# killerwhile/kafka-assignment-optimizer

Hardware: AMD Instinct MI355X
Metric: candidate assignments/sec (+ time_to_optimal_s), 10k-partition reassign (higher is better)
Workload: dtype int32

## Files before the change

kafka_assignment_optimizer_amd/csrc/kao_search.hip:

```cpp
#include "kao_search_dev.h"

namespace kao {

template <bool kGlobalA, bool kPriced, int NW, bool kWide, bool kTeam, bool kCurG = false, int RFT = 0, bool kSmall = false>
__device__ __forceinline__ void search_body(unsigned char *smem, const SearchPools &pl, const SearchParams &prm) {
    static_assert(!kTeam || kGlobalA, "teams run topics that live in global memory");
    static_assert(!kCurG || !kGlobalA, "kCurG: the working assignment is in LDS");
    static_assert(RFT == 0 || (RFT == 3 && NW == 4 && !kGlobalA && !kTeam), "RFT = 3: LDS-resident topics of four words per partition");
    static_assert(!kSmall || (RFT == 3 && !kPriced && !kCurG), "kSmall: the unpriced RF-3 instantiation");
    constexpr int NS = RFT ? RFT : NW;
    const int lane = threadIdx.x & 63;
    const int wave = __builtin_amdgcn_readfirstlane(threadIdx.x >> 6);
    const int n_waves = kTeam ? __builtin_amdgcn_readfirstlane((int)(blockDim.x >> 6)) : 1;
    const int tid = kTeam ? (int)threadIdx.x : lane, nthr = kTeam ? (int)blockDim.x : 64;
    const int2 bm = pl.block_map[blockIdx.x];
    const TopicDev *TD = pl.topics + bm.x;

    TopicRegs T = topic_regs<RFT>(TD);
    constexpr bool kBandTabs = kSmall;
    int bq_r0 = kBandTabs ? band_tab_bias(T.rep_lo) : T.rep_lo, bq_r1 = kBandTabs ? (int)band_tab(T.rep_lo, T.rep_hi) : T.rep_hi;
    int bq_l0 = kBandTabs ? band_tab_bias(T.lead_lo) : T.lead_lo, bq_l1 = kBandTabs ? (int)band_tab(T.lead_lo, T.lead_hi) : T.lead_hi;
    asm volatile("" : "+v"(bq_r0), "+v"(bq_r1), "+v"(bq_l0), "+v"(bq_l1));

    const int a_bytes = kGlobalA ? 0 : prm.maxP * NW * 4;
    const int cur_bytes = (kGlobalA || kCurG) ? 0 : prm.maxP * NW * 4;
    const int bx64 = (prm.maxBx + 63) & ~63;
    const int c_bytes = bx64 * 4;
    const int krt = search_rack_tab(prm.maxR);
    int *RSZ = reinterpret_cast<int *>(smem + cur_bytes);
    uint8_t *XR = smem + cur_bytes + krt * 4;
    const uint32_t inv = (uint32_t)krt - 1u;
    uint32_t *PR = reinterpret_cast<uint32_t *>(smem + cur_bytes + krt * 4 + bx64);
    const bool hbw = kPriced && prm.bw != 0;
    const int pr_bytes = kPriced ? (hbw ? 2 : 1) * c_bytes + krt * 4 : 0;
    int *PG = reinterpret_cast<int *>(smem + cur_bytes + krt * 4 + bx64 + c_bytes);
    uint32_t *BW = reinterpret_cast<uint32_t *>(smem + cur_bytes + krt * 4 + bx64 + c_bytes + krt * 4);
    unsigned char *wb = smem + cur_bytes + krt * 4 + bx64 + pr_bytes + (kTeam ? 0 : wave * (a_bytes + c_bytes + c_bytes / 2 + krt * 8));
    const Part<NW> *cur_words = reinterpret_cast<const Part<NW> *>(pl.cur_pool + TD->cur_off);
    const Part<NW> *CUR;
    if (kGlobalA || kCurG) CUR = cur_words; else CUR = reinterpret_cast<const Part<NW> *>(smem);
    WaveLds<NW> L;
    L.C = reinterpret_cast<uint32_t *>(wb + a_bytes);
    L.W = reinterpret_cast<uint16_t *>(wb + a_bytes + c_bytes);
    L.K = reinterpret_cast<int *>(wb + a_bytes + c_bytes + c_bytes / 2);
    L.RT = L.K + krt + (kTeam ? wave * krt : 0);
    int *TR = L.K + krt + n_waves * krt;
    int *TS = TR + 2 * 16 * kTeamRec;

    if (!kGlobalA && !kCurG) {
        Part<NW> *cur_lds = reinterpret_cast<Part<NW> *>(smem);
        for (int p = threadIdx.x; p < T.P; p += blockDim.x) cur_lds[p] = cur_words[p];
    }
    for (int r = threadIdx.x; r < krt; r += blockDim.x) {
        RSZ[r] = r < T.R ? pl.rsz_pool[TD->rsz_off + r] : 0;
        if (kPriced) PG[r] = r < T.R ? price_units(pl.price_pool[TD->price_off + 2 * TD->B + r], prm.obj_scale) : 0;
    }
    __syncthreads();
    for (int x = threadIdx.x; x < ((T.Bx + 63) & ~63); x += blockDim.x) {
        const uint32_t r = mulhi((uint32_t)x, T.magic);
        const bool valid = x < T.Bx && (int)((uint32_t)x - r * (uint32_t)T.m) < RSZ[r < (uint32_t)krt ? r : 0];
        XR[x] = valid ? (uint8_t)r : (uint8_t)inv;
        if (kPriced) {
            uint32_t pr = 0;
            if (valid) {
                const int32_t *pp = pl.price_pool + TD->price_off;
                const int b = pl.ext_pool[TD->ext_off + x];
                pr = ((uint32_t)price_units(pp[b], prm.obj_scale) & 0xFFFFu) | ((uint32_t)price_units(pp[TD->B + b], prm.obj_scale) << 16);
            }
            PR[x] = pr;
            if (hbw) BW[x] = (valid && TD->has_bw) ? pl.bw_pool[TD->bw_off + x] : 0u;
        }
    }
    __syncthreads();

    const int rho = bm.y + (kTeam ? 0 : wave);
    if (rho >= TD->n_restarts) return;
    const int g = TD->restart_base + rho;
    unsigned char *state_packed = pl.state_pool + TD->state_off + (uint64_t)rho * T.P * (NW * 2);
    if (kGlobalA) L.A = reinterpret_cast<Part<NW> *>(pl.state_pool + TD->state_off) + (uint64_t)rho * T.P;
    else L.A = reinterpret_cast<Part<NW> *>(wb);
    uint16_t *best = pl.best_pool + TD->best_off + (uint64_t)rho * T.P * T.RF;
    const uint16_t *ext = pl.ext_pool + TD->ext_off;
    const uint32_t slo = TD->seed_lo, shi = TD->seed_hi;
    const int S = prm.obj_scale;

    int best_obj, accepted;
    if (prm.init) {
        if (prm.init == 1)
        for (int p = tid; p < T.P; p += nthr) {
            Part<NW> c = CUR[p];
#pragma unroll
            for (int k = 1; k < NW; ++k)
                if (k >= T.RF) c.w[k] = kNoneW;
            L.A[p] = c;
        }
        best_obj = -1; accepted = 0;
    } else {
        best_obj = pl.restart_info[g * 4 + 0];
        accepted = pl.restart_info[g * 4 + 3];
        bool reseed = false;
        if (prm.elite) {
            const unsigned long long ek = pl.elite_key[bm.x];
            const int e_obj = (int)kObjCap - (int)((ek >> 20) & 0xFFFFFFull);
            reseed = ek != ~0ull && (ek >> 44) == 0 && (int)(ek & 0xFFFFFull) != rho && best_obj < e_obj &&
                     (fmix32(slo ^ ((uint32_t)rho * 0x9E3779B1u) ^ (prm.launch * 0x85EBCA77u) ^ 0xE117Eu) & 1u);
        }
        if (reseed) {
            const uint16_t *ea = pl.elite_assign + TD->win_off;
            const uint16_t *io = pl.int_pool + TD->int_off;
            for (int p = tid; p < T.P; p += nthr) {
                Part<NW> w;
#pragma unroll
                for (int k = 0; k < NW; ++k) w.w[k] = k < T.RF ? to_word(T, io[ea[p * T.RF + k]]) : kNoneW;
                L.A[p] = w;
            }
        } else if (!kGlobalA) {
            for (int p = lane; p < T.P; p += 64) L.A[p] = load_packed<NW>(T, state_packed, p);
        }
    }
    if (kGlobalA) __builtin_amdgcn_fence(__ATOMIC_SEQ_CST, "workgroup");
    if (kTeam) __syncthreads();
    recount(T, L, tid, nthr, krt);
    if (kTeam) __syncthreads();

    if (prm.init == 1) {
        const uint32_t *HL = pl.cur_pool + TD->hole_off;
        if (!kTeam || wave == 0)
        for (int pass = 0; pass < 2; ++pass) {
            const uint32_t n_holes = HL[pass], *hl = HL + 2 + (pass ? HL[0] : 0u);
            int p_n = n_holes ? (int)hl[0] : 0;
            Part<NW> a_n = L.A[p_n], c_n = CUR[p_n];
            for (uint32_t hi = 0; hi < n_holes; ++hi) {
                const int p = p_n;
                Part<NW> a = a_n;
                const Part<NW> c = c_n;
                if (hi + 1 < n_holes) { p_n = (int)hl[hi + 1]; a_n = L.A[p_n]; c_n = CUR[p_n]; }
#pragma unroll
                for (int k = 0; k < NW; ++k) {
                    if (k >= T.RF) break;
                    if ((k == 0) != (pass == 0)) continue;
                    if (a.w[k] != kNoneW) continue;
                    const uint32_t hmix = slo ^ fmix32(shi + (uint32_t)rho * 0x9E3779B1u + (uint32_t)(p * NW + k) * 0x27D4EB2Fu + 0x5BD1E995u + prm.gen * 0x632BE5ABu);
                    const int wl = k == 0 ? T.w00 : T.w01, wf = k == 0 ? T.w10 : T.w11;
                    uint32_t key = kKeyNull, xw_l = kNoneW;
#pragma unroll 2
                    for (int base = 0; base < T.Bx; base += 64) {
                        const uint32_t x = (uint32_t)(base + lane);
                        const uint32_t r = XR[x];
                        const uint32_t xw = x | (r << 16);
                        const bool okx = (r != inv) & !in4(a, xw);
                        const uint32_t cn = L.C[x];
                        const uint32_t rk = r;
                        int dV = dinc((int)(cn & 0xFFFFu), T.rep_lo, T.rep_hi) + dinc(L.K[rk], T.rack_lo, T.rack_hi) +
                                 dinc(cnt4(a, r), T.prack_lo, T.prack_hi);
                        if (k == 0) dV += dinc((int)(cn >> 16), T.lead_lo, T.lead_hi);
                        const uint32_t tie = fmix32(hmix + x * 0x165667B1u) >> 24;
                        uint32_t keyx;
                        if (kPriced) {
                            const uint32_t prx = PR[x];
                            int dP = p_in((int)(cn & 0xFFFFu), T.rep_lo, T.rep_hi, price_rep(prx)) + p_in(L.K[rk], T.rack_lo, T.rack_hi, PG[rk]);
                            if (k == 0) dP += p_in((int)(cn >> 16), T.lead_lo, T.lead_hi, price_lead(prx));
                            keyx = okx ? make_key_tie_p(prm.lam_max, S, dV, role_w2(c, xw, wl, wf) + (hbw ? bw_of(BW[x], k == 0) : 0), dP, tie) : kKeyNull;
                        }
                        else keyx = okx ? make_key_tie(prm.lam_max, S, dV, role_w2(c, xw, wl, wf), tie) : kKeyNull;
                        if (keyx < key) { key = keyx; xw_l = xw; }
                    }
                    const uint32_t kmin = wave_umin(key);
                    const unsigned long long bal = __ballot(key == kmin);
                    const uint32_t xw_win = (uint32_t)__builtin_amdgcn_readlane((int)xw_l, __ffsll((long long)bal) - 1);
                    a.w[k] = xw_win;
                    if (lane == 0) {
                        reinterpret_cast<uint32_t *>(&L.A[p])[k] = xw_win;
                        L.C[xw_win & 0xFFFFu] += (k == 0) ? 0x10001u : 1u;
                        L.K[xw_win >> 16] += 1;
                    }
                }
            }
        }
        if (kGlobalA) __builtin_amdgcn_fence(__ATOMIC_SEQ_CST, "workgroup");
        if (kTeam) __syncthreads();
    }

    int V, obj;
    full_cost<NW, kTeam>(T, L, CUR, RSZ, tid, nthr, V, obj, hbw ? BW : nullptr, TS, wave, n_waves);
    if (V == 0 && obj > best_obj) { best_obj = obj; snapshot(T, L, ext, best, tid, nthr); }
    rebuild_band_state(T, L, XR, inv, tid, nthr);
    if (lane == 0) L.RT[krt - 1] = 0;
    if (kTeam) __syncthreads();

    uint32_t rng = fmix32(slo ^ fmix32(shi + (uint32_t)rho * 0x9E3779B1u + prm.launch * 0x85EBCA77u + (uint32_t)tid * 0xC2B2AE3Du));

    const int plog = TD->period_log2 + (rho & 3);
    const uint32_t pmask = (1u << plog) - 1u;
    const uint32_t lrange = (uint32_t)(prm.lam_max - prm.lam_min + 1);
    const uint32_t RF8 = (uint32_t)T.RF << 8, R8 = (uint32_t)T.R << 8, m8 = (uint32_t)T.m << 8;

    const int T_tour = min(64, max(4, (T.P * T.RF) >> 2));
    uint32_t tour_off = lane < T_tour ? 0u : kKeyNull;
    asm volatile("" : "+v"(tour_off));
    const int GA = min(16, max(1, (T.P * T.RF) >> 8));
    const int x_rounds_full = (T.P + 63) >> 6;
    const bool x_windowed = x_rounds_full > 8;

    int lam_lo = prm.lam_min, lam_hi = prm.lam_max;
    uint32_t n_iters = prm.iters, it_base = prm.launch * prm.iters;
    constexpr uint32_t kLpScanTwo = 1u << 29;
    uint32_t loop_pack = TD->P * TD->RF <= prm.scan2_max ? kLpScanTwo : 0u;
    if (kSmall) loop_pack |= ((uint32_t)prm.lam_min & 0xFFFu) | (((uint32_t)prm.lam_max & 0xFFFu) << 12) | (((uint32_t)plog & 31u) << 24);
    {
        uint32_t v0 = (uint32_t)lam_lo, v1 = (uint32_t)lam_hi, v2 = n_iters, v3 = it_base, v4 = loop_pack;
        asm volatile("" : "+v"(v2), "+v"(v3), "+v"(v4));
        if constexpr (!kSmall) {
            asm volatile("" : "+v"(v0), "+v"(v1));
            lam_lo = (int)__builtin_amdgcn_readfirstlane(v0); lam_hi = (int)__builtin_amdgcn_readfirstlane(v1);
        }
        n_iters = __builtin_amdgcn_readfirstlane(v2); it_base = __builtin_amdgcn_readfirstlane(v3);
        loop_pack = __builtin_amdgcn_readfirstlane(v4);
    }
    auto loop_flag = [&](uint32_t bit) { uint32_t lp = loop_pack; asm volatile("" : "+s"(lp)); return (lp & bit) != 0u; };
    constexpr bool kFuse = !kGlobalA && !kTeam && !kPriced;
    const bool fuse_ok = kFuse && T.Bx <= 16384;
    uint32_t jmp_a = 1u, jmp_c = 0u;
    if (fuse_ok)
        for (int n = (T.Bx + 63) >> 6; n > 0; --n) { jmp_a = (jmp_a * 0x6D2B79u) & 0xFFFFFFu; jmp_c = (jmp_c * 0x6D2B79u + 0x3C6EF3u) & 0xFFFFFFu; }
    best_obj = __builtin_amdgcn_readfirstlane(best_obj);
    for (uint32_t i = 0; i < n_iters; ++i) {
        const uint32_t it = it_base + i;
        const int type = (int)((0x1210u >> ((it & 7u) * 2u)) & 3u);
        int lam;
        if constexpr (kSmall) {
            uint32_t lp = loop_pack;
            asm volatile("" : "+s"(lp));
            const uint32_t plg = (lp >> 24) & 31u;
            const int lo_ = (int)(lp & 0xFFFu), hi_ = (int)((lp >> 12) & 0xFFFu);
            const uint32_t ph = it & ((1u << plg) - 1u);
            lam = best_obj < 0 ? hi_ : min(hi_, lo_ + (int)((2u * ph * (uint32_t)(hi_ - lo_ + 1)) >> plg));
        } else {
            const uint32_t ph = it & pmask;
            lam = best_obj < 0 ? lam_hi : min(lam_hi, lam_lo + (int)((2u * ph * lrange) >> plog));
        }
        const bool sampled = (type == 2) || (type == 0 && ((it >> 3) & 1u));

        auto finish = [&](auto ty, auto uni, uint32_t kmin, int win, int p, int k, int q, int j, uint32_t uw, uint32_t vw, int dV, int dObj) {
            constexpr int TY = decltype(ty)::value;
            auto of_win = [&](int v) { return decltype(uni)::value ? v : __builtin_amdgcn_readlane(v, win); };
            if (!kTeam) {
                if (kmin == kKeyNull) return;
                if ((int)(kmin >> 8) - kDBias > 0) return;
            }
            bool mine = true;
            int *rec = TR + ((i & 1u) * 16 + (uint32_t)wave) * kTeamRec;
            if (kTeam) {
                const bool ok = kmin != kKeyNull && (int)(kmin >> 8) - kDBias <= 0;
                if (lane == win) {
                    const uint32_t ro_ = uw >> 16, rn_ = vw >> 16;
                    const bool racks = ok && TY == 0 && ro_ != rn_;
                    rec[0] = ok ? 1 : 0; rec[1] = p; rec[2] = TY == 1 ? q : p;
                    rec[3] = (int)(uw & 0xFFFFu); rec[4] = (int)(vw & 0xFFFFu);
                    rec[5] = racks ? (int)ro_ : 0xFFFF; rec[6] = racks ? (int)rn_ : 0xFFFF;
                    rec[7] = dV; rec[8] = dObj;
                }
                __syncthreads();
                bool clash = false;
                if (lane < wave) {
                    const int *o = TR + ((i & 1u) * 16 + (uint32_t)lane) * kTeamRec;
                    if (o[0]) {
                        const int mp = rec[1], mq = rec[2], mb0 = rec[3], mb1 = rec[4], mr0 = rec[5], mr1 = rec[6];
                        clash = (o[1] == mp) | (o[1] == mq) | (o[2] == mp) | (o[2] == mq) | (o[3] == mb0) | (o[3] == mb1) | (o[4] == mb0) | (o[4] == mb1);
                        if (o[5] != 0xFFFF && mr0 != 0xFFFF) clash |= (o[5] == mr0) | (o[5] == mr1) | (o[6] == mr0) | (o[6] == mr1);
                    }
                }
                mine = ok && __ballot(clash) == 0ull;
            }

            if (lane == win && mine) {
                uint32_t *ap = reinterpret_cast<uint32_t *>(&L.A[p]);
                if (TY == 0) {
                    const uint32_t d = (k == 0) ? 0x10001u : 1u;
                    L.C[uw & 0xFFFFu] -= d;
                    L.C[vw & 0xFFFFu] += d;
                    if (!kTeam || (uw >> 16) != (vw >> 16)) {
                        L.K[uw >> 16] -= 1;
                        L.K[vw >> 16] += 1;
                    }
                    ap[k] = vw;
                } else if (TY == 1) {
                    uint32_t *bp = reinterpret_cast<uint32_t *>(&L.A[q]);
                    if ((k == 0) != (j == 0)) {
                        const uint32_t lose = (k == 0) ? uw : vw, gain = (k == 0) ? vw : uw;
                        L.C[lose & 0xFFFFu] -= 0x10000u;
                        L.C[gain & 0xFFFFu] += 0x10000u;
                    }
                    ap[k] = vw;
                    bp[j] = uw;
                } else {
                    L.C[uw & 0xFFFFu] -= 0x10000u;
                    L.C[vw & 0xFFFFu] += 0x10000u;
                    ap[0] = vw;
                    ap[k] = uw;
                }
            }
            if (mine) {
                int rows;
                if (TY == 0) rows = 1 | (of_win(k) == 0 ? 2 : 0);
                else if (TY == 1) rows = (of_win(k) == 0 ? 2 : 0) ^ (of_win(j) == 0 ? 2 : 0);
                else rows = 2;
                if (rows != 0) {
                    const uint32_t xo = (uint32_t)of_win((int)uw) & 0xFFFFu, xn = decltype(uni)::value ? (uint32_t)__builtin_amdgcn_readfirstlane((int)(vw & 0xFFFFu)) : (uint32_t)of_win((int)vw) & 0xFFFFu;
                    uint32_t xx = xo;
                    asm("v_writelane_b32 %0, %1, 1" : "+v"(xx) : "s"(xn));
                    int lane_w = lane;
                    asm volatile("" : "+v"(lane_w));
                    if (lane_w < 2) {
                        const uint32_t cx = L.C[xx];
                        uint32_t wx;
                        if (rows == 3) wx = band_row<kBandTabs>((int)(cx & 0xFFFFu), bq_r0, bq_r1) | (band_row<kBandTabs>((int)(cx >> 16), bq_l0, bq_l1) << 6);
                        else if (rows == 1) wx = (L.W[xx] & ~kWRowR) | band_row<kBandTabs>((int)(cx & 0xFFFFu), bq_r0, bq_r1);
                        else wx = (L.W[xx] & ~kWRowL) | (band_row<kBandTabs>((int)(cx >> 16), bq_l0, bq_l1) << 6);
                        L.W[xx] = (uint16_t)wx;
                    }
                }
            }
            if (kGlobalA) __builtin_amdgcn_fence(__ATOMIC_SEQ_CST, "workgroup");
            if (kTeam) {
                if (lane == 0) rec[9] = mine ? 1 : 0;
                __syncthreads();
                int dVs = 0, dOs = 0, na = 0;
                if (lane < n_waves) {
                    const int *o = TR + ((i & 1u) * 16 + (uint32_t)lane) * kTeamRec;
                    if (o[9]) { dVs = o[7]; dOs = o[8]; na = 1; }
                }
                V += wave_sum(dVs);
                obj += wave_sum(dOs);
                accepted += wave_sum(na);
            } else {
                V += of_win(dV);
                obj += of_win(dObj);
                accepted++;
            }
        };
        constexpr std::integral_constant<int, 0> kReplace{};
        constexpr std::integral_constant<int, 1> kExchange{};
        constexpr std::integral_constant<int, 2> kLeaderSwap{};

        if (sampled) {
            const int p = (int)rnd24_wide(rng, (uint32_t)T.P);
            const Part<NW> a = L.A[p];
            const Part<NW> c = CUR[p];
            uint32_t key = kKeyNull, vw = 0;
            int dV = 0, dObj = 0;
            if (type == 0) {
                const int k = (int)rnd24(rng, RF8);
                const uint32_t uw = sel_slot<NS>(a, k);
                const uint32_t ro = uw >> 16;
                const bool lead = k == 0;
                const uint32_t lw = lead ? 2u : 0u;
                const int wl = lead ? T.w00 : T.w01, wf = lead ? T.w10 : T.w11;
                const int g_old = role_w2<NS>(c, uw, wl, wf) + (hbw ? bw_of(BW[uw & 0xFFFFu], lead) : 0);
                const uint32_t wo = L.W[uw & 0xFFFFu];
                const int dV_old = wfld(wo, kWDecR) + wfldw(wo, kWDecL, lw);
                const int dV_rack_old = ddec(L.K[ro], T.rack_lo, T.rack_hi) + c7_delta(T.c7_dec, cnt4x2<NS>(a, ro));
                const int rsz_ro = RSZ[ro];
                int dP_old = 0, dP_rack_old = 0;
                if (kPriced) {
                    const uint32_t pro = PR[uw & 0xFFFFu];
                    dP_old = -(wflag(wo, kWPoutR) & price_rep(pro));
                    if (lead) dP_old -= wflag(wo, kWPoutL) & price_lead(pro);
                    dP_rack_old = p_out(L.K[ro], T.rack_lo, T.rack_hi, PG[ro]);
                }
                const int base_s = kSmall ? mad24s(S, g_old, kDBias) : 0;
#pragma unroll
                for (int g = 0; g < 4; ++g) {
                    uint32_t r, jj;
                    bool okg;
                    if (g < 2) {
                        r = rnd24(rng, R8);
                        jj = rnd24(rng, m8);
                        okg = (int)jj < RSZ[r];
                    } else {
                        r = ro;
                        jj = rnd24(rng, (uint32_t)rsz_ro << 8);
                        okg = true;
                    }
                    const uint32_t x = __umul24(r, (uint32_t)T.m) + jj;
                    const uint32_t xw = x | (r << 16);
                    okg = okg && !in4<NS>(a, xw);
                    const uint32_t wn = L.W[x];
                    int dVg = dV_old + wfld(wn, kWIncR) + wfldw(wn, kWIncL, lw);
                    if (g < 2) {
                        if (r != ro)
                            dVg += dV_rack_old + dinc(L.K[r], T.rack_lo, T.rack_hi) + c7_delta(T.c7_inc, cnt4x2<NS>(a, r));
                    }
                    const int dObjg = role_w2<NS>(c, xw, wl, wf) + (hbw ? bw_of(BW[x], lead) : 0) - (kSmall ? 0 : g_old);
                    uint32_t keyg;
                    if constexpr (kSmall) keyg = okg ? key_small(mad24s(-S, dObjg, mad24s(lam, dVg, base_s)), (uint32_t)lane) : kKeyNull;
                    else if (kPriced) {
                        const uint32_t prx = PR[x];
                        int dPg = dP_old + (wflag(wn, kWPinR) & price_rep(prx));
                        if (lead) dPg += wflag(wn, kWPinL) & price_lead(prx);
                        if (g < 2 && r != ro) dPg += dP_rack_old + p_in(L.K[r], T.rack_lo, T.rack_hi, PG[r]);
                        keyg = okg ? make_key_p(lam, S, dVg, dObjg, dPg, lane) : kKeyNull;
                    }
                    else keyg = okg ? make_key(lam, S, dVg, dObjg, lane) : kKeyNull;
                    if (keyg < key) { key = keyg; vw = xw; dV = dVg; dObj = dObjg; }
                }
                if constexpr (kSmall) dObj -= g_old;
                const uint32_t kmin = wave_umin(key);
                finish(kReplace, std::false_type{}, kmin, (int)(kmin & 63u), p, k, 0, 0, uw, vw, dV, dObj);
            } else {
                const uint32_t uw = a.w[0];
                int k = 0;
                const int u_lead = role_w2<NS>(c, uw, T.w00, T.w10), u_fol = role_w2<NS>(c, uw, T.w01, T.w11);
                const uint32_t wu = L.W[uw & 0xFFFFu];
                const int dV_u = wfld(wu, kWDecL);
                const int dP_u = kPriced ? -(wflag(wu, kWPoutL) & price_lead(PR[uw & 0xFFFFu])) : 0;
#pragma unroll
                for (int kk = 1; kk < NS; ++kk) {
                    if (!RFT && kk >= T.RF) break;
                    const uint32_t xw = a.w[kk];
                    const int dObjg = role_w2<NS>(c, xw, T.w00, T.w10) + u_fol - u_lead - role_w2<NS>(c, xw, T.w01, T.w11) +
                                      (hbw ? (int)(BW[xw & 0xFFFFu] >> 16) - (int)(BW[uw & 0xFFFFu] >> 16) : 0);
                    const uint32_t wx = L.W[xw & 0xFFFFu];
                    const int dVg = dV_u + wfld(wx, kWIncL);
                    uint32_t keyg;
                    if constexpr (kSmall) keyg = key_small(mad24s(lam, dVg, mad24s(-S, dObjg, kDBias)), (uint32_t)lane);
                    else if (kPriced) keyg = make_key_p(lam, S, dVg, dObjg, dP_u + (wflag(wx, kWPinL) & price_lead(PR[xw & 0xFFFFu])), lane);
                    else keyg = make_key(lam, S, dVg, dObjg, lane);
                    if (keyg < key) { key = keyg; vw = xw; k = kk; dV = dVg; dObj = dObjg; }
                }
                const uint32_t kmin = wave_umin(key);
                finish(kLeaderSwap, std::false_type{}, kmin, (int)(kmin & 63u), p, k, 0, 0, uw, vw, dV, dObj);
            }
        } else {
            uint32_t keyA, oldw_l;
            int pl_, kl_, g_old_l, dvo_l = 0, dvr_l = 0;
            auto score_words = [&](auto ty, uint32_t &key_o, const Part<NW> &al, const Part<NW> &cl, int k_o, uint32_t &oldw_o, int &g_o, int &dvo_o, int &dvr_o) {
                constexpr int TY = decltype(ty)::value;
                oldw_o = sel_slot<NS>(al, k_o);
                const uint32_t rol = oldw_o >> 16;
                const bool leadl = k_o == 0;
                g_o = role_w2<NS>(cl, oldw_o, leadl ? T.w00 : T.w01, leadl ? T.w10 : T.w11);
                if (hbw && TY == 0) g_o += bw_of(BW[oldw_o & 0xFFFFu], leadl);
                const uint32_t wo = L.W[oldw_o & 0xFFFFu];
                const int dv7 = c7_delta(T.c7_dec, cnt4x2<NS>(al, rol));
                int sc;
                if (TY == 0) {
                    dvo_o = wfld(wo, kWDecR) + wfldw(wo, kWDecL, leadl ? 2u : 0u);
                    dvr_o = ddec(L.K[rol], T.rack_lo, T.rack_hi) + dv7;
                    sc = dvo_o + min(dvr_o, 0);
                } else {
                    const int dvl = wfld(wo, leadl ? kWDecL : kWIncL);
                    sc = min(dv7, 0) + min(dvl, 0);
                }
                if constexpr (kSmall) key_o = key_small(mad24s(lam, sc, mad24s(S, g_o, kDBias)), (uint32_t)lane) | tour_off;
                else if (kPriced) {
                    int dPs = 0;
                    if (TY == 0) {
                        const uint32_t pro = PR[oldw_o & 0xFFFFu];
                        dPs = -(wflag(wo, kWPoutR) & price_rep(pro));
                        dPs -= wflagw(wo, kWPoutL, leadl ? 1u : 0u) & price_lead(pro);
                    }
                    key_o = make_key_p(lam, S, sc, -g_o, dPs, lane) | tour_off;
                }
                else key_o = make_key(lam, S, sc, -g_o, lane) | tour_off;
            };
            auto score_slot = [&](auto ty, uint32_t &key_o, int p_o, int &k_o, uint32_t &oldw_o, int &g_o, int &dvo_o, int &dvr_o) {
                k_o = (int)rnd24(rng, RF8);
                const Part<NW> al = L.A[p_o];
                const Part<NW> cl = CUR[p_o];
                score_words(ty, key_o, al, cl, k_o, oldw_o, g_o, dvo_o, dvr_o);
            };
            auto tournament = [&](auto ty) {
                const int p0 = (int)rnd24_wide(rng, (uint32_t)T.P);
                auto part = [&](int ga) { const int q2 = p0 + ga; return q2 < T.P ? q2 : q2 - T.P; };
                pl_ = p0;
                score_slot(ty, keyA, p0, kl_, oldw_l, g_old_l, dvo_l, dvr_l);
                int ga = 1;
                for (; kWide && ga + 1 < GA; ga += 2) {
                    uint32_t kg0, ow0, kg1, ow1;
                    int kk0, gg0, d10 = 0, d20 = 0, kk1, gg1, d11 = 0, d21 = 0;
                    const int pg0 = part(ga), pg1 = part(ga + 1);
                    score_slot(ty, kg0, pg0, kk0, ow0, gg0, d10, d20);
                    score_slot(ty, kg1, pg1, kk1, ow1, gg1, d11, d21);
                    if (kg0 < keyA) { keyA = kg0; pl_ = pg0; kl_ = kk0; oldw_l = ow0; g_old_l = gg0; dvo_l = d10; dvr_l = d20; }
                    if (kg1 < keyA) { keyA = kg1; pl_ = pg1; kl_ = kk1; oldw_l = ow1; g_old_l = gg1; dvo_l = d11; dvr_l = d21; }
                }
                for (; ga < GA; ++ga) {
                    uint32_t kg, ow;
                    int kk, gg, d1 = 0, d2 = 0;
                    const int pg = part(ga);
// ... 708 lines not shown
```

kafka_assignment_optimizer_amd/csrc/kao_search_dev.h:

```cpp
#pragma once
#include <hip/hip_runtime.h>

#include <type_traits>

#include "kao_device.h"
#include "kao_internal.h"

namespace kao {

__device__ __forceinline__ uint32_t fmix32(uint32_t h) {
    h ^= h >> 16; h *= 0x85EBCA6Bu; h ^= h >> 13; h *= 0xC2B2AE35u; h ^= h >> 16;
    return h;
}
__device__ __forceinline__ uint32_t xs32(uint32_t &s) {
    s ^= s << 13; s ^= s >> 17; s ^= s << 5;
    return s;
}
__device__ __forceinline__ uint32_t mulhi(uint32_t a, uint32_t b) { return __umulhi(a, b); }
__device__ __forceinline__ int band(int c, int lo, int hi) { return max(c - hi, 0) + max(lo - c, 0); }
__device__ __forceinline__ int dinc(int c, int lo, int hi) { return (int)(c >= hi) - (int)(c < lo); }
__device__ __forceinline__ int ddec(int c, int lo, int hi) { return (int)(c <= lo) - (int)(c > hi); }

template <int NW> struct alignas(16) Part { uint32_t w[NW]; };
__device__ __forceinline__ uint32_t sel4(const Part<4> &a, int k) {
    const uint32_t lo = (k & 2) ? a.w[2] : a.w[0];
    const uint32_t hi = (k & 2) ? a.w[3] : a.w[1];
    return (k & 1) ? hi : lo;
}
__device__ __forceinline__ uint32_t sel4(const Part<8> &a, int k) {
    const uint32_t q0 = (k & 4) ? a.w[4] : a.w[0], q1 = (k & 4) ? a.w[5] : a.w[1], q2 = (k & 4) ? a.w[6] : a.w[2], q3 = (k & 4) ? a.w[7] : a.w[3];
    const uint32_t lo = (k & 2) ? q2 : q0, hi = (k & 2) ? q3 : q1;
    return (k & 1) ? hi : lo;
}
template <int NW> __device__ __forceinline__ void set_slot(Part<NW> &a, int k, uint32_t v) {
#pragma unroll
    for (int i = 0; i < NW; ++i) a.w[i] = (i == k) ? v : a.w[i];
}
__device__ __forceinline__ uint32_t lcg24(uint32_t &s) {
    asm("v_mad_u32_u24 %0, %0, %1, %2" : "+v"(s) : "s"(0x6D2B79u), "v"(0x3C6EF3u));
    return s;
}
__device__ __forceinline__ uint32_t rnd24(uint32_t &s, uint32_t n8) {
    const uint32_t v = lcg24(s);
    return (uint32_t)(((unsigned long long)(v & 0xFFFFFFu) * (unsigned long long)(n8 & 0xFFFFFFu)) >> 32);
}
__device__ __forceinline__ uint32_t rnd24_wide(uint32_t &s, uint32_t n) {
    const uint32_t v = lcg24(s);
    return __umulhi((v & 0xFFFFFFu) << 8, n);
}
__device__ __forceinline__ uint32_t key_of(int delta, uint32_t low) {
    delta = min(max(delta, -kDBias), kDBias - 2);
    return ((uint32_t)(delta + kDBias) << 8) | low;
}
__device__ __forceinline__ uint32_t make_key_p(int lam, int S, int dV, int dObj, int dP, int lane) { return key_of(__mul24(lam, dV) - __mul24(S, dObj) + dP, (uint32_t)lane); }
__device__ __forceinline__ uint32_t make_key(int lam, int S, int dV, int dObj, int lane) { return key_of(__mul24(lam, dV) - __mul24(S, dObj), (uint32_t)lane); }
__device__ __forceinline__ uint32_t make_key_tie_p(int lam, int S, int dV, int dObj, int dP, uint32_t tie) { return key_of(__mul24(lam, dV) - __mul24(S, dObj) + dP, tie & 0xFFu); }
__device__ __forceinline__ uint32_t make_key_tie(int lam, int S, int dV, int dObj, uint32_t tie) { return key_of(__mul24(lam, dV) - __mul24(S, dObj), tie & 0xFFu); }
__device__ __forceinline__ int mad24(int a, int b, int c) {
    int r;
    asm("v_mad_i32_i24 %0, %1, %2, %3" : "=v"(r) : "v"(a), "v"(b), "v"(c));
    return r;
}
__device__ __forceinline__ int mad24s(int s, int b, int c) {
    int r;
    asm("v_mad_i32_i24 %0, %1, %2, %3" : "=v"(r) : "s"(s), "v"(b), "v"(c));
    return r;
}
__device__ __forceinline__ uint32_t key_small(int biased_cost, uint32_t low) { return ((uint32_t)biased_cost << 8) | low; }
__device__ __forceinline__ uint32_t pk_mad_lo(uint32_t a, uint32_t b, uint32_t c) {
    uint32_t r;
    asm("v_pk_mad_i16 %0, %1, %2, %3 op_sel_hi:[0,1,0]" : "=v"(r) : "v"(a), "v"(b), "v"(c));
    return r;
}
__device__ __forceinline__ uint32_t pk_mad_s(uint32_t a, uint32_t s, uint32_t c) {
    uint32_t r;
    asm("v_pk_mad_i16 %0, %1, %2, %3 op_sel_hi:[1,0,1]" : "=v"(r) : "v"(a), "v"(s), "v"(c));
    return r;
}
__device__ __forceinline__ uint32_t pk_mad_ss(uint32_t a, uint32_t s, uint32_t c) {
    uint32_t r;
    asm("v_pk_mad_i16 %0, %1, %2, %3 op_sel_hi:[1,0,1]" : "=v"(r) : "v"(a), "s"(s), "v"(c));
    return r;
}
__device__ __forceinline__ uint32_t pk_add(uint32_t a, uint32_t b) {
    uint32_t r;
    asm("v_pk_add_i16 %0, %1, %2" : "=v"(r) : "v"(a), "v"(b));
    return r;
}
__device__ __forceinline__ uint32_t pk_sub(uint32_t a, uint32_t b) {
    uint32_t r;
    asm("v_pk_sub_i16 %0, %1, %2" : "=v"(r) : "v"(a), "v"(b));
    return r;
}
__device__ __forceinline__ int price_rep(uint32_t pr) { return (int)(short)(pr & 0xFFFFu); }
__device__ __forceinline__ int price_lead(uint32_t pr) { return (int)pr >> 16; }
__device__ __forceinline__ int p_in(int c, int lo, int hi, int price) { return ((c >= hi) | (c < lo)) ? price : 0; }
__device__ __forceinline__ int p_out(int c, int lo, int hi, int price) { return ((c > hi) | (c <= lo)) ? -price : 0; }
__device__ __forceinline__ int bw_of(uint32_t bw, bool lead) { return (int)(bw & 0xFFFFu) + (lead ? (int)(bw >> 16) : 0); }
__device__ __forceinline__ int price_units(int v, int S) { return min(max((S * v + kDualScale / 2) >> kDualLog2, -32767), 32767); }

template <int NS = 0, int NW> __device__ __forceinline__ bool in4(const Part<NW> &a, uint32_t w) {
    bool r = false;
#pragma unroll
    for (int i = 0; i < (NS ? NS : NW); ++i) r |= a.w[i] == w;
    return r;
}
template <int NS = 0, int NW> __device__ __forceinline__ int cnt4(const Part<NW> &a, uint32_t r) {
    int n = 0;
#pragma unroll
    for (int i = 0; i < (NS ? NS : NW); ++i) n += (int)((a.w[i] >> 16) == r);
    return n;
}
template <int NS = 0, int NW> __device__ __forceinline__ int cnt4x2(const Part<NW> &a, uint32_t r) { return cnt4<NS>(a, r) << 1; }
template <int NS, int NW> __device__ __forceinline__ uint32_t sel_slot(const Part<NW> &a, int k) {
    if constexpr (NS == 3 && NW == 4) {
        int k1 = k & 1, k2 = k & 2;
        asm("" : "+v"(k1), "+v"(k2));
        const uint32_t w0 = a.w[0], w1 = a.w[1], w2 = a.w[2];
        return k2 ? w2 : (k1 ? w1 : w0);
    } else return sel4(a, k);
}

constexpr uint32_t c7_tab(bool dec, int lo, int hi) {
    uint32_t t = 0;
    for (int c = 0; c <= 8; ++c) {
        const int d = dec ? (c <= lo ? 1 : 0) - (c > hi ? 1 : 0) : (c >= hi ? 1 : 0) - (c < lo ? 1 : 0);
        t |= ((uint32_t)d & 3u) << (2 * c);
    }
    return t;
}
__device__ __forceinline__ int c7_delta(uint32_t tab, int cnt2) { return __builtin_amdgcn_sbfe((int)tab, (unsigned)cnt2, 2u); }

struct TopicRegs {
    int P, RF, R, m, Bx;
    uint32_t magic;
    int rep_lo, rep_hi, lead_lo, lead_hi, rack_lo, rack_hi, prack_lo, prack_hi;
    int w00, w01, w10, w11;
    uint32_t c7_inc, c7_dec;
};

template <int RFT = 0> __device__ __forceinline__ TopicRegs topic_regs(const TopicDev *TD) {
    TopicRegs T;
    T.P = TD->P; T.RF = RFT ? RFT : TD->RF; T.R = TD->R; T.m = TD->m; T.Bx = TD->Bx; T.magic = TD->magic;
    T.rep_lo = TD->rep_lo; T.rep_hi = TD->rep_hi; T.lead_lo = TD->lead_lo; T.lead_hi = TD->lead_hi;
    T.rack_lo = TD->rack_lo; T.rack_hi = TD->rack_hi; T.prack_lo = TD->prack_lo; T.prack_hi = TD->prack_hi;
    T.w00 = TD->w00; T.w01 = TD->w01; T.w10 = TD->w10; T.w11 = TD->w11;
    T.c7_inc = c7_tab(false, T.prack_lo, T.prack_hi); T.c7_dec = c7_tab(true, T.prack_lo, T.prack_hi);
    return T;
}

template <int NS = 0, int NW> __device__ __forceinline__ int role_w2(const Part<NW> &c, uint32_t w, int wl, int wf) {
    bool fol = false;
#pragma unroll
    for (int i = 1; i < (NS ? NS : NW); ++i) fol |= c.w[i] == w;
    return (c.w[0] == w) ? wl : (fol ? wf : 0);
}
template <int NS = 0, int NW> __device__ __forceinline__ int role_w(const TopicRegs &T, const Part<NW> &c, uint32_t w, int nr) {
    return role_w2<NS>(c, w, nr ? T.w01 : T.w00, nr ? T.w11 : T.w10);
}
__device__ __forceinline__ uint32_t to_word(const TopicRegs &T, uint32_t x) {
    return x == 0xFFFFu ? kNoneW : (x | (mulhi(x, T.magic) << 16));
}
template <int NW> __device__ __forceinline__ Part<NW> load_packed(const TopicRegs &T, const unsigned char *base, int p) {
    Part<NW> a;
    if (NW == 4) {
        const uint2 s = reinterpret_cast<const uint2 *>(base)[p];
        a.w[0] = to_word(T, s.x & 0xFFFFu); a.w[1] = to_word(T, s.x >> 16); a.w[2] = to_word(T, s.y & 0xFFFFu); a.w[3] = to_word(T, s.y >> 16);
    } else {
        const uint4 s = reinterpret_cast<const uint4 *>(base)[p];
        const uint32_t v[4] = {s.x, s.y, s.z, s.w};
#pragma unroll
        for (int i = 0; i < NW / 2; ++i) { a.w[2 * i] = to_word(T, v[i & 3] & 0xFFFFu); a.w[2 * i + 1] = to_word(T, v[i & 3] >> 16); }
    }
    return a;
}
template <int NW> __device__ __forceinline__ void store_packed(unsigned char *base, int p, const Part<NW> &a) {
    if (NW == 4) reinterpret_cast<uint2 *>(base)[p] = make_uint2((a.w[0] & 0xFFFFu) | (a.w[1] << 16), (a.w[2] & 0xFFFFu) | (a.w[3] << 16));
    else reinterpret_cast<uint4 *>(base)[p] = make_uint4((a.w[0] & 0xFFFFu) | (a.w[1] << 16), (a.w[2] & 0xFFFFu) | (a.w[3] << 16),
                                                         (a.w[4 % NW] & 0xFFFFu) | (a.w[5 % NW] << 16), (a.w[6 % NW] & 0xFFFFu) | (a.w[7 % NW] << 16));
}
template <int NW> __device__ __forceinline__ int part_rack_viol(const TopicRegs &T, const Part<NW> &a) {
    int s = 0, touched = 0;
#pragma unroll
    for (int k = 0; k < NW; ++k) {
        const uint32_t rk = a.w[k] >> 16;
        bool first = a.w[k] != kNoneW;
#pragma unroll
        for (int j = 0; j < k; ++j) first &= (a.w[j] >> 16) != rk;
        if (first) { s += band(cnt4(a, rk), T.prack_lo, T.prack_hi); touched++; }
    }
    return s + (T.R - touched) * T.prack_lo;
}

constexpr int kTeamRec = 12;
template <int NW> struct WaveLds {
    Part<NW> *A;
    uint32_t *C;
    uint16_t *W;
    int *K;
    int *RT;
};

constexpr int kWIncR = 0, kWDecR = 2, kWPinR = 4, kWPoutR = 5, kWIncL = 6, kWDecL = 8, kWPinL = 10, kWPoutL = 11;
__device__ __forceinline__ int wfld(uint32_t w, int off) { return __builtin_amdgcn_sbfe((int)w, (unsigned)off, 2u); }
__device__ __forceinline__ int wfldw(uint32_t w, int off, uint32_t width) { return __builtin_amdgcn_sbfe((int)w, (unsigned)off, width); }
__device__ __forceinline__ int wflag(uint32_t w, int off) { return __builtin_amdgcn_sbfe((int)w, (unsigned)off, 1u); }
__device__ __forceinline__ int wflagw(uint32_t w, int off, uint32_t width) { return __builtin_amdgcn_sbfe((int)w, (unsigned)off, width); }
constexpr unsigned long long band_entry_of(int a, int b) {
    const int di = (b >= 0 ? 1 : 0) - (a < 0 ? 1 : 0), dd = (a <= 0 ? 1 : 0) - (b > 0 ? 1 : 0);
    const int pin = (b >= 0 || a < 0) ? 1 : 0, pout = (b > 0 || a <= 0) ? 1 : 0;
    return (unsigned long long)((di & 3) | ((dd & 3) << 2) | (pin << 4) | (pout << 5));
}
constexpr unsigned long long band_table() {
    unsigned long long t = 0;
    for (int a = -1; a <= 1; ++a) for (int b = -1; b <= 1; ++b) t |= band_entry_of(a, b) << (6 * (3 * (a + 1) + (b + 1)));
    return t;
}
constexpr unsigned long long kBandTab = band_table();
__device__ __forceinline__ int clamp_pm1(int x) {
    int r;
    asm("v_med3_i32 %0, %1, -1, 1" : "=v"(r) : "v"(x));
    return r;
}
__device__ __forceinline__ uint32_t band_entry(int c, int lo, int hi) {
    const int a = clamp_pm1(c - lo), b = clamp_pm1(c - hi);
    int t;
    asm("v_mad_i32_i24 %0, %1, 3, %2" : "=v"(t) : "v"(a), "v"(b));
    return (uint32_t)(kBandTab >> (uint32_t)(__mul24(t, 6) + 24)) & 63u;
}
constexpr int kBandTabLast = 4;
constexpr bool band_tab_fits(int lo, int hi) { return lo >= 0 && lo <= hi && hi <= 0xFFFF && hi - lo + 2 <= kBandTabLast; }
constexpr uint32_t band_tab(int lo, int hi) {
    uint32_t t = 0;
    for (int i = 0; i <= kBandTabLast; ++i) {
        const int c = lo - 1 + (i < hi - lo + 2 ? i : hi - lo + 2);
        const int a = c < lo ? -1 : (c > lo ? 1 : 0), b = c < hi ? -1 : (c > hi ? 1 : 0);
        t |= (uint32_t)band_entry_of(a, b) << (6 * i);
    }
    return t;
}
constexpr int band_tab_bias(int lo) { return 6 - 6 * lo; }
constexpr uint32_t band_lookup_plain(int c, int bias, uint32_t tab) {
    const int x = 6 * c + bias;
    return (tab >> (x < 0 ? 0 : (x > 6 * kBandTabLast ? 6 * kBandTabLast : x))) & 63u;
}
__device__ __forceinline__ uint32_t band_lookup(int c, int bias, uint32_t tab) {
    int x;
    asm("v_mad_i32_i24 %0, %1, 6, %2\n\tv_med3_i32 %0, %0, 0, 24" : "=&v"(x) : "v"(c), "v"(bias));
    static_assert(6 * kBandTabLast == 24, "the clamp's inline constant");
    return __builtin_amdgcn_ubfe(tab, (uint32_t)x, 6u);
}
template <bool kTab> __device__ __forceinline__ uint32_t band_row(int c, int r0, int r1) {
    if constexpr (kTab) return band_lookup(c, r0, (uint32_t)r1);
    else return band_entry(c, r0, r1);
}
__device__ __forceinline__ uint32_t band_fields(const TopicRegs &T, uint32_t c) {
    return band_entry((int)(c & 0xFFFFu), T.rep_lo, T.rep_hi) | (band_entry((int)(c >> 16), T.lead_lo, T.lead_hi) << 6);
}
constexpr uint32_t kWRowR = 0x003Fu, kWRowL = 0x0FC0u;
constexpr uint32_t kWNoCand = 0x8000u;
constexpr uint32_t kWNoCand2 = 0x4000u;
template <int NW> __device__ __forceinline__ void rebuild_band_state(const TopicRegs &T, const WaveLds<NW> &L, const uint8_t *XR, uint32_t inv, int lane, int stride = 64) {
    for (int x = lane; x < ((T.Bx + 63) & ~63); x += stride) L.W[x] = (uint16_t)(XR[x] == inv ? (kWNoCand | kWNoCand2) : band_fields(T, L.C[x]));
}

template <int NW> __device__ __forceinline__ void recount(const TopicRegs &T, const WaveLds<NW> &L, int lane, int stride, int krt) {
    for (int x = lane; x < ((T.Bx + 63) & ~63); x += stride) L.C[x] = 0;
    for (int r = lane; r < krt; r += stride) L.K[r] = 0;
    if (stride > 64) __syncthreads();
    for (int p = lane; p < T.P; p += stride) {
        const Part<NW> a = L.A[p];
#pragma unroll
        for (int k = 0; k < NW; ++k)
            if (a.w[k] != kNoneW) { atomicAdd(&L.C[a.w[k] & 0xFFFFu], k == 0 ? 0x10001u : 1u); atomicAdd(&L.K[a.w[k] >> 16], 1); }
    }
}

template <int NW, bool kTeam = false> __device__ __forceinline__ void full_cost(const TopicRegs &T, const WaveLds<NW> &L, const Part<NW> *CUR, const int *RSZ,
                                                            int lane, int stride, int &V, int &obj, const uint32_t *BW = nullptr,
                                                            int *TS = nullptr, int wave = 0, int n_waves = 1) {
    int v = 0, o = 0;
    for (int p = lane; p < T.P; p += stride) {
        const Part<NW> a = L.A[p];
        const Part<NW> c = CUR[p];
#pragma unroll
        for (int k = 0; k < NW; ++k)
            if (a.w[k] != kNoneW) o += role_w(T, c, a.w[k], k == 0 ? 0 : 1);
        v += part_rack_viol(T, a);
    }
    for (int x = lane; x < T.Bx; x += stride) {
        const int r = (int)mulhi((uint32_t)x, T.magic);
        if (x - r * T.m < RSZ[r]) {
            const uint32_t c = L.C[x];
            v += band((int)(c & 0xFFFFu), T.rep_lo, T.rep_hi) + band((int)(c >> 16), T.lead_lo, T.lead_hi);
            if (BW) { const uint32_t bw = BW[x]; o += (int)(c & 0xFFFFu) * (int)(bw & 0xFFFFu) + (int)(c >> 16) * (int)(bw >> 16); }
        }
    }
    for (int r = lane; r < T.R; r += stride) v += band(L.K[r], T.rack_lo, T.rack_hi);
    V = wave_sum(v);
    obj = wave_sum(o);
    if (kTeam) {
        __syncthreads();
        if ((lane & 63) == 0) { TS[2 * wave] = V; TS[2 * wave + 1] = obj; }
        __syncthreads();
        int tv = 0, to = 0;
        if ((lane & 63) < n_waves) { tv = TS[2 * (lane & 63)]; to = TS[2 * (lane & 63) + 1]; }
        V = wave_sum(tv);
        obj = wave_sum(to);
    }
}

template <int NW> __device__ __forceinline__ void snapshot(const TopicRegs &T, const WaveLds<NW> &L, const uint16_t *ext, uint16_t *best, int lane, int stride = 64) {
    for (int p0 = 0; p0 < T.P; p0 += stride) {
        const int p = p0 + lane;
        if (p < T.P) {
            const Part<NW> a = L.A[p];
            uint16_t *o = best + p * T.RF;
#pragma unroll
            for (int k = 0; k < NW; ++k)
                if (k < T.RF) o[k] = ext[a.w[k] & 0xFFFFu];
        }
    }
}

}
```

Measured before the change: 886.0 billion.

## Rewrite hole-fill init to use cached band state and per-rack delta table

Moves the band-state rebuild ahead of hole filling so the init pass can reuse the packed per-broker band words (L.W) and a per-hole rack delta table instead of recomputing dinc/price terms from raw counts for every candidate. Candidate scoring is split into a shared fill_round helper that packs cost, tie hash and round index into one key. The role-weight term is evaluated only in rounds that hold the partition's current replicas. Brokers already in the partition are marked in L.W rather than tested per candidate, and the band words are updated incrementally after each placement. This adds per-hole table builds and mark/unmark LDS writes, and it changes tie-breaking and key packing, so the chosen assignments can differ from the old path.

```diff
diff --git a/kafka_assignment_optimizer_amd/csrc/kao_search.hip b/kafka_assignment_optimizer_amd/csrc/kao_search.hip
--- a/kafka_assignment_optimizer_amd/csrc/kao_search.hip
+++ b/kafka_assignment_optimizer_amd/csrc/kao_search.hip
@@ -17,6 +17,11 @@
     const TopicDev *TD = pl.topics + bm.x;
 
     TopicRegs T = topic_regs<RFT>(TD);
+    {
+        uint32_t v0 = T.c7_inc, v1 = T.c7_dec;
+        asm volatile("" : "+v"(v0), "+v"(v1));
+        T.c7_inc = (uint32_t)__builtin_amdgcn_readfirstlane((int)v0); T.c7_dec = (uint32_t)__builtin_amdgcn_readfirstlane((int)v1);
+    }
     constexpr bool kBandTabs = kSmall;
     int bq_r0 = kBandTabs ? band_tab_bias(T.rep_lo) : T.rep_lo, bq_r1 = kBandTabs ? (int)band_tab(T.rep_lo, T.rep_hi) : T.rep_hi;
     int bq_l0 = kBandTabs ? band_tab_bias(T.lead_lo) : T.lead_lo, bq_l1 = kBandTabs ? (int)band_tab(T.lead_lo, T.lead_hi) : T.lead_hi;
@@ -123,8 +128,14 @@
     recount(T, L, tid, nthr, krt);
     if (kTeam) __syncthreads();
 
+    rebuild_band_state(T, L, XR, inv, tid, nthr);
+    if (lane == 0) L.RT[krt - 1] = 0;
+    if (kTeam) __syncthreads();
+
     if (prm.init == 1) {
+        constexpr bool kFillWeights = RFT != 3;
         const uint32_t *HL = pl.cur_pool + TD->hole_off;
+        const FillTabs F{L.W, XR, L.K, L.RT, PR, PG, hbw ? BW : nullptr};
         if (!kTeam || wave == 0)
         for (int pass = 0; pass < 2; ++pass) {
             const uint32_t n_holes = HL[pass], *hl = HL + 2 + (pass ? HL[0] : 0u);
@@ -135,46 +146,27 @@
                 Part<NW> a = a_n;
                 const Part<NW> c = c_n;
                 if (hi + 1 < n_holes) { p_n = (int)hl[hi + 1]; a_n = L.A[p_n]; c_n = CUR[p_n]; }
-#pragma unroll
-                for (int k = 0; k < NW; ++k) {
-                    if (k >= T.RF) break;
-                    if ((k == 0) != (pass == 0)) continue;
-                    if (a.w[k] != kNoneW) continue;
+                fill_mark<NS>(L.W, a, lane);
+#pragma nounroll
+                for (int k = pass; k < (pass ? T.RF : 1); ++k) {
+                    if ((uint32_t)__builtin_amdgcn_readfirstlane((int)sel_slot<NS>(a, k)) != kNoneW) continue;
                     const uint32_t hmix = slo ^ fmix32(shi + (uint32_t)rho * 0x9E3779B1u + (uint32_t)(p * NW + k) * 0x27D4EB2Fu + 0x5BD1E995u + prm.gen * 0x632BE5ABu);
-                    const int wl = k == 0 ? T.w00 : T.w01, wf = k == 0 ? T.w10 : T.w11;
-                    uint32_t key = kKeyNull, xw_l = kNoneW;
-#pragma unroll 2
-                    for (int base = 0; base < T.Bx; base += 64) {
-                        const uint32_t x = (uint32_t)(base + lane);
-                        const uint32_t r = XR[x];
-                        const uint32_t xw = x | (r << 16);
-                        const bool okx = (r != inv) & !in4(a, xw);
-                        const uint32_t cn = L.C[x];
-                        const uint32_t rk = r;
-                        int dV = dinc((int)(cn & 0xFFFFu), T.rep_lo, T.rep_hi) + dinc(L.K[rk], T.rack_lo, T.rack_hi) +
-                                 dinc(cnt4(a, r), T.prack_lo, T.prack_hi);
-                        if (k == 0) dV += dinc((int)(cn >> 16), T.lead_lo, T.lead_hi);
-                        const uint32_t tie = fmix32(hmix + x * 0x165667B1u) >> 24;
-                        uint32_t keyx;
-                        if (kPriced) {
-                            const uint32_t prx = PR[x];
-                            int dP = p_in((int)(cn & 0xFFFFu), T.rep_lo, T.rep_hi, price_rep(prx)) + p_in(L.K[rk], T.rack_lo, T.rack_hi, PG[rk]);
-                            if (k == 0) dP += p_in((int)(cn >> 16), T.lead_lo, T.lead_hi, price_lead(prx));
-                            keyx = okx ? make_key_tie_p(prm.lam_max, S, dV, role_w2(c, xw, wl, wf) + (hbw ? bw_of(BW[x], k == 0) : 0), dP, tie) : kKeyNull;
-                        }
-                        else keyx = okx ? make_key_tie(prm.lam_max, S, dV, role_w2(c, xw, wl, wf), tie) : kKeyNull;
-                        if (keyx < key) { key = keyx; xw_l = xw; }
-                    }
-                    const uint32_t kmin = wave_umin(key);
-                    const unsigned long long bal = __ballot(key == kmin);
-                    const uint32_t xw_win = (uint32_t)__builtin_amdgcn_readlane((int)xw_l, __ffsll((long long)bal) - 1);
-                    a.w[k] = xw_win;
+                    const uint32_t xw_win = fill_hole<NS, kPriced, !kSmall, kFillWeights>(T, F, a, c, k == 0, hmix, prm.lam_max, S, lane);
+                    if (xw_win == kNoneW) continue;
+                    set_slot(a, k, xw_win);
                     if (lane == 0) {
+                        const uint32_t xs = xw_win & 0xFFFFu;
                         reinterpret_cast<uint32_t *>(&L.A[p])[k] = xw_win;
-                        L.C[xw_win & 0xFFFFu] += (k == 0) ? 0x10001u : 1u;
+                        const uint32_t cx = L.C[xs] + ((k == 0) ? 0x10001u : 1u);
+                        L.C[xs] = cx;
                         L.K[xw_win >> 16] += 1;
-                    }
-                }
+                        uint32_t wx = band_row<kBandTabs>((int)(cx & 0xFFFFu), bq_r0, bq_r1);
+                        if (k == 0) wx |= band_row<kBandTabs>((int)(cx >> 16), bq_l0, bq_l1) << 6;
+                        else wx |= L.W[xs] & kWRowL;
+                        L.W[xs] = (uint16_t)(wx | kWNoCand);
+                    }
+                }
+                fill_unmark<NS>(L.W, a, lane);
             }
         }
         if (kGlobalA) __builtin_amdgcn_fence(__ATOMIC_SEQ_CST, "workgroup");
@@ -184,8 +176,6 @@
     int V, obj;
     full_cost<NW, kTeam>(T, L, CUR, RSZ, tid, nthr, V, obj, hbw ? BW : nullptr, TS, wave, n_waves);
     if (V == 0 && obj > best_obj) { best_obj = obj; snapshot(T, L, ext, best, tid, nthr); }
-    rebuild_band_state(T, L, XR, inv, tid, nthr);
-    if (lane == 0) L.RT[krt - 1] = 0;
     if (kTeam) __syncthreads();
 
     uint32_t rng = fmix32(slo ^ fmix32(shi + (uint32_t)rho * 0x9E3779B1u + prm.launch * 0x85EBCA77u + (uint32_t)tid * 0xC2B2AE3Du));
diff --git a/kafka_assignment_optimizer_amd/csrc/kao_search_dev.h b/kafka_assignment_optimizer_amd/csrc/kao_search_dev.h
--- a/kafka_assignment_optimizer_amd/csrc/kao_search_dev.h
+++ b/kafka_assignment_optimizer_amd/csrc/kao_search_dev.h
@@ -262,6 +262,94 @@
 constexpr uint32_t kWNoCand2 = 0x4000u;
 template <int NW> __device__ __forceinline__ void rebuild_band_state(const TopicRegs &T, const WaveLds<NW> &L, const uint8_t *XR, uint32_t inv, int lane, int stride = 64) {
     for (int x = lane; x < ((T.Bx + 63) & ~63); x += stride) L.W[x] = (uint16_t)(XR[x] == inv ? (kWNoCand | kWNoCand2) : band_fields(T, L.C[x]));
+}
+
+struct FillTabs {
+    uint16_t *W;
+    const uint8_t *XR;
+    const int *K;
+    int *RT;
+    const uint32_t *PR;
+    const int *PG;
+    const uint32_t *BW;
+};
+constexpr uint32_t kFillTieStep = 0x165667B1u;
+template <int NS, int NW> __device__ __forceinline__ void fill_mark(uint16_t *W, const Part<NW> &a, int lane) {
+    const uint32_t ai = sel_slot<NS>(a, lane & (NW - 1));
+    if ((lane < NS) & (ai != kNoneW)) W[ai & 0xFFFFu] |= (uint16_t)kWNoCand;
+}
+template <int NS, int NW> __device__ __forceinline__ void fill_unmark(uint16_t *W, const Part<NW> &a, int lane) {
+    const uint32_t ai = sel_slot<NS>(a, lane & (NW - 1));
+    if ((lane < NS) & (ai != kNoneW)) W[ai & 0xFFFFu] &= (uint16_t)~kWNoCand;
+}
+template <int NS, bool kPriced, int NW> __device__ __forceinline__ void fill_rack_table(const TopicRegs &T, const FillTabs &F, const Part<NW> &a, int lane) {
+    for (int r = lane; r < T.R; r += 64) {
+        const int kr = F.K[r];
+        int v = dinc(kr, T.rack_lo, T.rack_hi) + c7_delta(T.c7_inc, cnt4x2<NS>(a, (uint32_t)r));
+        if (kPriced) v = (v & 0xFF) | (p_in(kr, T.rack_lo, T.rack_hi, F.PG[r]) * 256);
+        F.RT[r] = v;
+    }
+}
+template <int NS, bool kPriced, bool kClamp, bool kWithW, int NW>
+__device__ __forceinline__ uint32_t fill_round(const TopicRegs &T, const FillTabs &F, const Part<NW> &c, int x, int rd, uint32_t h, int lam, int S, bool lead) {
+    const int w = (int)reinterpret_cast<const short *>(F.W)[x];
+    const uint32_t r = F.XR[x];
+    const int rt = F.RT[r];
+    const uint32_t lw = lead ? 2u : 0u, lf = lead ? 1u : 0u;
+    int cost;
+    if (kPriced) {
+        const uint32_t prx = F.PR[x];
+        const int dVx = wfld(w, kWIncR) + wfldw(w, kWIncL, lw) + (int)(signed char)(rt & 0xFF);
+        cost = __mul24(lam, dVx) + kDBias + (rt >> 8) + (wflag(w, kWPinR) & price_rep(prx)) + (wflagw(w, kWPinL, lf) & price_lead(prx));
+        if (F.BW) cost -= __mul24(S, bw_of(F.BW[x], lead));
+    } else {
+        cost = mad24s(lam, wfld(w, kWIncR) + wfldw(w, kWIncL, lw) + rt, kDBias);
+    }
+    if (kWithW) cost -= __mul24(S, role_w2<NS>(c, (uint32_t)x | (r << 16), lead ? T.w00 : T.w01, lead ? T.w10 : T.w11));
+    if (kClamp) cost = min(max(cost, 0), 2 * kDBias - 2);
+    h ^= h >> 16; h *= 0x85EBCA6Bu; h ^= h >> 13; h *= 0xC2B2AE35u;
+    return ((uint32_t)cost << 16) | ((h >> 16) & 0xFF00u) | (uint32_t)rd | ((uint32_t)w & 0xFFFF0000u);
+}
+template <int NS, bool kPriced, bool kClamp, bool kWeights, int NW>
+__device__ __forceinline__ uint32_t fill_hole(const TopicRegs &T, const FillTabs &F, const Part<NW> &a, const Part<NW> &c, bool lead, uint32_t hmix, int lam, int S, int lane) {
+    fill_rack_table<NS, kPriced>(T, F, a, lane);
+    int mr[NS] = {};
+    if constexpr (kWeights) {
+        const uint32_t ci = sel_slot<NS>(c, lane & (NW - 1));
+        const int mr_l = ((lane < NS) & (ci != kNoneW) & !in4<NS>(a, ci)) ? (int)((ci & 0xFFFFu) >> 6) : -1;
+#pragma unroll
+        for (int i = 0; i < NS; ++i) mr[i] = __builtin_amdgcn_readlane(mr_l, i);
+    }
+    uint32_t h = hmix + (uint32_t)lane * kFillTieStep;
+    uint32_t best = kKeyNull;
+    int chunk = 0;
+    for (int cb = 0; cb < T.Bx; cb += 16384) {
+        uint32_t bestc = kKeyNull;
+        const int n_rd = (min(T.Bx, cb + 16384) - cb + 63) >> 6;
+        int rd = 0, x = cb + lane;
+        if constexpr (!kWeights) {
+            for (; rd + 1 < n_rd; rd += 2, x += 128, h += 128u * kFillTieStep) {
+                const uint32_t k0 = fill_round<NS, kPriced, kClamp, false>(T, F, c, x, rd, h, lam, S, lead);
+                const uint32_t k1 = fill_round<NS, kPriced, kClamp, false>(T, F, c, x + 64, rd + 1, h + 64u * kFillTieStep, lam, S, lead);
+                bestc = min(bestc, min(k0, k1));
+            }
+            if (rd < n_rd) { bestc = min(bestc, fill_round<NS, kPriced, kClamp, false>(T, F, c, x, rd, h, lam, S, lead)); h += 64u * kFillTieStep; }
+        } else {
+            for (; rd < n_rd; ++rd, x += 64, h += 64u * kFillTieStep) {
+                bool wgt = false;
+#pragma unroll
+                for (int i = 0; i < NS; ++i) wgt |= mr[i] == (cb >> 6) + rd;
+                bestc = min(bestc, wgt ? fill_round<NS, kPriced, kClamp, true>(T, F, c, x, rd, h, lam, S, lead) : fill_round<NS, kPriced, kClamp, false>(T, F, c, x, rd, h, lam, S, lead));
+            }
+        }
+        if ((bestc >> 8) < (best >> 8)) { best = bestc; chunk = cb; }
+    }
+    const uint32_t m = wave_umin(((best >> 1) & ~127u) | (uint32_t)lane);
+    if ((m >> 15) == 0xFFFFu) return kNoneW;
+    const int win = (int)(m & 63u);
+    const uint32_t bw = (uint32_t)__builtin_amdgcn_readlane((int)best, win);
+    const uint32_t xs = (uint32_t)__builtin_amdgcn_readlane(chunk, win) + ((bw & 255u) << 6) + (uint32_t)win;
+    return xs | ((uint32_t)F.XR[xs] << 16);
 }
 
 template <int NW> __device__ __forceinline__ void recount(const TopicRegs &T, const WaveLds<NW> &L, int lane, int stride, int krt) {
@@ -311,7 +399,8 @@
 }
 
 template <int NW> __device__ __forceinline__ void snapshot(const TopicRegs &T, const WaveLds<NW> &L, const uint16_t *ext, uint16_t *best, int lane, int stride = 64) {
-    for (int p0 = 0; p0 < T.P; p0 += stride) {
+    int p0 = 0;
+    do {
         const int p = p0 + lane;
         if (p < T.P) {
             const Part<NW> a = L.A[p];
@@ -320,7 +409,8 @@
             for (int k = 0; k < NW; ++k)
                 if (k < T.RF) o[k] = ext[a.w[k] & 0xFFFFu];
         }
-    }
-}
-
-}
+        p0 += stride;
+    } while (p0 < T.P);
+}
+
+}
```

New measurement: 907.6 billion, median of 6. 1.02x the previous value.
